# tudocomp/tudocomp

Measured on AMD Instinct MI355X. Metric: input MB/s end-to-end lcpcomp+huffman, higher is better.
Workload: dtype u32; 1 GPU; lcpcomp(coder=huff,threshold=2,flatten=1,comp=arrays) on 2000000000 B english text (SURVEY 8d generator, seed 42): pinned host text -> H2D -> kernels + host Huffman table -> D2H -> stream in pinned host memory, all timed; bytes_per_gpu=2000000000, parallelism=single GPU

## Files before the change

### tudocomp_amd/csrc/api_ctx.hip

```cpp
#include "api.hpp"
#include "huffman_host.hpp"

#include <strings.h>
#include <ctype.h>

using namespace tdc;

namespace tdc {

int lcpcomp_enc_coder(int coder) {
    const int base = coder & 0xFF, k = coder >> 8;
    if (base == TDC_GPU_CODER_SLE) {
        if (k < 0 || k > 7) throw ArgError{TDC_GPU_ERR_ARG, "sle: kmer must be in 1..7"};
        return 3 | ((k ? k : 3) << 8);
    }
    if (k == 0 && base == TDC_GPU_CODER_HUFF) return 0;
    if (k == 0 && base == TDC_GPU_CODER_ARITH) return 1;
    if (k == 0 && base == TDC_GPU_CODER_ASCII) return 2;
    throw ArgError{TDC_GPU_ERR_UNSUPPORTED, "lcpcomp: coder must be huff, arithmetic, ascii or sle"};
}

void reserve_arena(Ctx& c, size_t bytes) {
    if (c.arena.size < bytes) {
        size_t fr = 0, tot = 0;
// ... 23 lines not shown
        case TDC_GPU_ERR_UNSUPPORTED: return "No implementation found for this coder/strategy";
        case TDC_GPU_ERR_INTERNAL: return "internal error";
        default: return "unknown status";
    }
}

const char* tdc_gpu_last_error(const tdc_gpu_ctx* ctx) { return ctx ? ctx->last_error.c_str() : ""; }

void tdc_gpu_free(void* p) { free(p); }

namespace {
struct OptionDef { const char* name; void (*set)(Ctx&, long); };
inline int clampi(long v, long lo, long hi) { return (int)(v < lo ? lo : (v > hi ? hi : v)); }
const OptionDef OPTIONS[] = {
    { "fastread",         [](Ctx& c, long v) { c.fast_read = v ? 1 : 0; } },
    { "sa_local",         [](Ctx& c, long v) { c.sa_local_sort = (int)v; } },
    { "radix_waves",      [](Ctx& c, long v) { c.radix_waves = v == 8 ? 8 : 4; } },
    { "window_lcut",      [](Ctx& c, long v) { c.window_lcut = clampi(v, 0, 63); } },
    { "window_halo",      [](Ctx& c, long v) { c.window_halo = clampi(v, 0, 2048); } },
    { "dec_seg",          [](Ctx& c, long v) { c.dec_seg = v < 4096 ? 4096 : (v > (1l << 30) ? (size_t)1 << 30 : (size_t)v); } },
    { "dec_lean",         [](Ctx& c, long v) { c.dec_lean = v != 0; } },
    { "dec_parse",        [](Ctx& c, long v) { c.dec_parse = clampi(v, 0, 2); } },
    { "dec_done",         [](Ctx& c, long v) { c.dec_done = v != 0; } },
    { "dec_log",          [](Ctx& c, long v) { c.dec_log = v != 0; } },
    { "bwt_log",          [](Ctx& c, long v) { c.bwt_log = v != 0; } },
    { "pipe_log",         [](Ctx& c, long v) { c.pipe_log = v != 0; } },
    { "window_force_fail",[](Ctx& c, long v) { c.window_force_fail = v ? 1 : 0; } },
    { "window_large",     [](Ctx& c, long v) { c.window_large_lists = v ? 1 : 0; } },
    { "window_src",       [](Ctx& c, long v) { c.window_src = v ? 1 : 0; } },
    { "plcp_samples",     [](Ctx& c, long v) { c.plcp_samples = v != 0; } },
    { "small_pipeline",   [](Ctx& c, long v) { c.small_pipeline = v != 0; } },
    { "small_big",        [](Ctx& c, long v) { c.small_big = (int)v; } },
    { "small_prof",       [](Ctx& c, long v) { c.small_prof = v != 0; } },
    { "phi_lazy",         [](Ctx& c, long v) { c.phi_lazy = v != 0; } },
    { "fs_pair",          [](Ctx& c, long v) { c.fs_pair = v != 0; } },
    { "enc_early",        [](Ctx& c, long v) { c.enc_early = (int)v; } },
    { "owner_rem",        [](Ctx& c, long v) { c.owner_rem = (int)std::min<long>(std::max<long>(v, 0), 8); } },
    { "enc_rec",          [](Ctx& c, long v) { c.enc_rec = v != 0; } },
    { "level_purge",      [](Ctx& c, long v) { c.level_purge = v != 0; } },
    { "level_log",        [](Ctx& c, long v) { c.level_log = v != 0; } },
    { "eager",            [](Ctx& c, long v) { c.eager_levels = v != 0; } },
    { "eager_dump",       [](Ctx& c, long v) { c.eager_dump = v != 0; } },
    { "flen_bytes",       [](Ctx& c, long v) { c.flen_bytes = v != 0; } },
    { "flatten_steps",    [](Ctx& c, long v) { c.flatten_steps = v <= 0 ? (1 << 30) : clampi(v, 1, 1 << 30); } },
    { "flatten_growth",   [](Ctx& c, long v) { c.flatten_growth = clampi(v, 2, 1 << 20); } },
    { "sa_refine",        [](Ctx& c, long v) { c.sa_refine = v != 0; } },
    { "sa_pairs",         [](Ctx& c, long v) { c.sa_pairs = v != 0; } },
    { "sa_stars",         [](Ctx& c, long v) { c.sa_stars = v != 0; } },
    { "sa_fused_init",    [](Ctx& c, long v) { c.sa_fused_init = v != 0; } },
    { "sa_init_syms",     [](Ctx& c, long v) { c.sa_init_syms = clampi(v, 0, 64); } },
    { "radix_lds",        [](Ctx& c, long v) { c.radix_lds = (v >= 0 && v <= 2) ? (int)v : 2; } },
    { "xcd_remap",        [](Ctx& c, long v) { c.xcd_remap = (v >= 0 && v <= 2) ? (int)v : 0; } },
    { "bucket_scatter",   [](Ctx& c, long v) { c.bucket_scatter = v ? 1 : 0; } },
    { "ssort",            [](Ctx& c, long v) { c.ssort = v ? 1 : 0; } },
    { "ssort_levels",     [](Ctx& c, long v) { c.ssort_levels = (v >= 1 && v <= 3) ? (int)v : 0; } },
    { "msd_partition",    [](Ctx& c, long v) { c.msd_partition = v ? 1 : 0; } },
    { "wsort",            [](Ctx& c, long v) { c.wsort = v ? 1 : 0; } },
    { "wsort_min",        [](Ctx& c, long v) { c.wsort_min = v < 4096 ? 4096 : (size_t)v; } },
    { "wsort_syms",       [](Ctx& c, long v) { c.wsort_syms = (v >= 4 && v <= 64) ? (int)v : 0; } },
    { "wsort_kw",         [](Ctx& c, long v) { c.wsort_kw = (v == 1 || v == 2) ? (int)v : 0; } },
    { "wsort_rounds",     [](Ctx& c, long v) { c.wsort_rounds = clampi(v, 0, 100); } },
    { "wsort_smallrun",   [](Ctx& c, long v) { c.wsort_small = v ? 1 : 0; } },
    { "wsort_overlap",    [](Ctx& c, long v) { c.wsort_overlap = v ? 1 : 0; } },
    { "wsort_predig",     [](Ctx& c, long v) { c.wsort_predig = v ? 1 : 0; } },
    { "wsort_prehist",    [](Ctx& c, long v) { c.wsort_prehist = v ? 1 : 0; } },
    { "sa_seg_bigcap",    [](Ctx& c, long v) { c.sa_seg_bigcap = clampi(v, 0, 65536); } },
    { "sa_seg_rounds",    [](Ctx& c, long v) { c.sa_seg_rounds = clampi(v, 0, 2); } },
    { "wsort_run_streams",[](Ctx& c, long v) { c.wsort_run_streams = v != 0; } },
    { "wsort_predig_skip",[](Ctx& c, long v) { c.wsort_predig_skip = clampi(v, 0, 24); } },
    { "wsort_fuse",       [](Ctx& c, long v) { c.wsort_fuse = v ? 1 : 0; } },
    { "wsort_order",      [](Ctx& c, long v) { c.wsort_order = v ? 1 : 0; } },
    { "wsort_two",        [](Ctx& c, long v) { c.wsort_two = (v >= 0 && v <= 2) ? (int)v : 0; } },
    { "wsort_leaf",       [](Ctx& c, long v) { c.wsort_leaf = v == 1024 ? 1024 : 2048; } },
    { "wsort_pack",       [](Ctx& c, long v) { c.wsort_pack = (v == 1024 || v == 4096) ? (int)v : 2048; } },
    { "wsort_cmax",       [](Ctx& c, long v) { c.wsort_cmax = clampi(v, 8, 64); } },
    { "wsort_log",        [](Ctx& c, long v) { c.wsort_log = v != 0; } },
    { "upload_chunks",    [](Ctx& c, long v) { c.upload_chunks = clampi(v, 4, 24); } },
    { "upload_tail_n",    [](Ctx& c, long v) { c.upload_tail_n = clampi(v, 0, 12); } },
    { "upload_tail_pct",  [](Ctx& c, long v) { c.upload_tail_pct = clampi(v, 30, 100); } },
    { "arena_log",        [](Ctx& c, long v) { c.arena_log = v != 0; } },
};
constexpr size_t NOPTIONS = sizeof(OPTIONS) / sizeof(OPTIONS[0]);
const OptionDef FOLD_OPTIONS[] = {
    { "fused_cand",       [](Ctx& c, long v) { c.fused_cand = v != 0; } },
    { "sel_tile_counts",  [](Ctx& c, long v) { c.sel_tile_counts = v != 0; } },
    { "flatten_chunks",   [](Ctx& c, long v) { c.flatten_chunks = clampi(v, 0, (long)FLATTEN_MAX_CHUNKS); } },
    { "repair_recount",   [](Ctx& c, long v) { c.repair_recount = v != 0; } },
    { "repair_table_bits",[](Ctx& c, long v) { c.repair_table_bits = v == 0 ? 0 : clampi(v, 8, 30); } },
    { "repair_log",       [](Ctx& c, long v) { c.repair_log = v != 0; } },
};
constexpr size_t NFOLD = sizeof(FOLD_OPTIONS) / sizeof(FOLD_OPTIONS[0]);
const OptionDef* find_option(const char* name) {
    if (!name) return nullptr;
    if (!strncasecmp(name, "TDC_GPU_", 8)) name += 8;
    for (size_t i = 0; i < NOPTIONS; ++i) if (!strcasecmp(name, OPTIONS[i].name)) return &OPTIONS[i];
    for (size_t i = 0; i < NFOLD; ++i) if (!strcasecmp(name, FOLD_OPTIONS[i].name)) return &FOLD_OPTIONS[i];
    return nullptr;
}
void apply_env_options(tdc_gpu_ctx* ctx) {
    const char* on = getenv("TDC_GPU_DEBUG_KNOBS");
    if (!on || atoi(on) == 0) return;
    for (size_t i = 0; i < NOPTIONS + NFOLD; ++i) {
        const OptionDef& o = i < NOPTIONS ? OPTIONS[i] : FOLD_OPTIONS[i - NOPTIONS];
        char var[64] = "TDC_GPU_";
        size_t k = 8;
        for (const char* q = o.name; *q && k + 1 < sizeof(var); ++q) var[k++] = (char)toupper((unsigned char)*q);
        var[k] = 0;
        if (const char* m = getenv(var)) o.set(ctx->c, atol(m));
    }
}
}

int tdc_gpu_ctx_set_option(tdc_gpu_ctx* ctx, const char* name, long value) {
    if (!ctx) return TDC_GPU_ERR_ARG;
    const OptionDef* o = find_option(name);
    if (!o) return TDC_GPU_ERR_ARG;
    o->set(ctx->c, value);
    return TDC_GPU_OK;
}
int tdc_gpu_option_count(void) { return (int)NOPTIONS; }
const char* tdc_gpu_option_name(int i) { return (i >= 0 && (size_t)i < NOPTIONS) ? OPTIONS[i].name : nullptr; }

int tdc_gpu_ctx_create(int device, tdc_gpu_ctx** out) {
    if (!out) return TDC_GPU_ERR_ARG;
    *out = nullptr;
    int count = 0;
    if (hipGetDeviceCount(&count) != hipSuccess || count <= 0) { (void)hipGetLastError(); return TDC_GPU_ERR_HIP; }
    if (device < 0 || device >= count) return TDC_GPU_ERR_ARG;
    tdc_gpu_ctx* ctx = new (std::nothrow) tdc_gpu_ctx();
    if (!ctx) return TDC_GPU_ERR_OOM;
    ctx->c.huff_ok = huffman_selfcheck();
    ctx->c.device = device;
    ctx->c.wpre = &ctx->pre;
    DeviceGuard dg(device);
    try {
        HIP_TRY(dg.enter());
        HIP_TRY(hipStreamCreateWithFlags(&ctx->c.stream, hipStreamNonBlocking));
        for (auto& e : ctx->c.ev) HIP_TRY(hipEventCreate(&e));
        HIP_TRY(hipStreamCreateWithFlags(&ctx->c.copy_stream, hipStreamNonBlocking));
        {
            int lo = 0, hi = 0;
            if (hipDeviceGetStreamPriorityRange(&lo, &hi) != hipSuccess) { lo = 0; (void)hipGetLastError(); }
            if (hipStreamCreateWithPriority(&ctx->c.aux_stream, hipStreamNonBlocking, lo) != hipSuccess) { ctx->c.aux_stream = nullptr; (void)hipGetLastError(); }
        }
        HIP_TRY(hipEventCreateWithFlags(&ctx->c.ev_join, hipEventDisableTiming));
        HIP_TRY(hipEventCreateWithFlags(&ctx->c.ev_dig2, hipEventDisableTiming));
        for (auto& e : ctx->c.ev_chunk) HIP_TRY(hipEventCreateWithFlags(&e, hipEventDisableTiming));
        ctx->c.pinned_size = 4096;
        HIP_TRY(hipHostMalloc(&ctx->c.pinned, ctx->c.pinned_size, hipHostMallocDefault));
        HIP_TRY(hipHostMalloc((void**)&ctx->c.pinned_hdr, Ctx::PINNED_HDR, hipHostMallocDefault));
        if (ctx->c.fast_read) {
            void* zc = nullptr;
            if (hipHostMalloc(&zc, (size_t)Ctx::ZC_WORDS * Ctx::ZC_BLOCKS * 4, hipHostMallocMapped | hipHostMallocCoherent) == hipSuccess) {
                void* dv = nullptr;
                if (hipHostGetDevicePointer(&dv, zc, 0) == hipSuccess) { ctx->c.zc_host = (u32*)zc; ctx->c.zc_dev = (u32*)dv; memset(zc, 0, (size_t)Ctx::ZC_WORDS * Ctx::ZC_BLOCKS * 4); }
                else { (void)hipHostFree(zc); (void)hipGetLastError(); }
            } else (void)hipGetLastError();
        }
        HIP_TRY(hipMalloc((void**)&ctx->c.d_err, 256));
        HIP_TRY(hipMemset(ctx->c.d_err, 0, 256));
        apply_env_options(ctx);
    } catch (const HipError&) {
        (void)hipGetLastError();
        tdc_gpu_ctx_destroy(ctx);
        return TDC_GPU_ERR_HIP;
    }
// ... 142 lines not shown
```

### tudocomp_amd/csrc/common.hpp

```cpp
#pragma once

#include <hip/hip_runtime.h>
#include <stdint.h>
#include <stddef.h>
#include <stdio.h>
#include <string.h>

namespace tdc {

typedef uint8_t  u8;
typedef uint32_t u32;
typedef uint16_t u16;
typedef uint64_t u64;

constexpr u32 NONE32 = 0xFFFFFFFFu;
constexpr int WAVE = 64;

enum {
    TDC_OK = 0,
    TDC_ERR_HIP = -1,
    TDC_ERR_ARG = -2,
    TDC_ERR_NO_SENTINEL = -3,
    TDC_ERR_TOO_LARGE = -4,
    TDC_ERR_OOM = -5,
// ... 44 lines not shown
    }
    template <typename T> T* get_top(size_t count) { return (T*)alloc_top(count * sizeof(T)); }
    void release_top() { top_hi = 0; }
    size_t mark() const { return top; }
    void release(size_t m) { top = m; }
};

enum KernelClass {
    K_RS_SCATTER_U64 = 0, K_RS_SCATTER_U32, K_RS_COUNT, K_SCAN,
    K_SA_RANK_SCATTER, K_SA_BUILD_KEYS, K_PHI, K_PLCP, K_CAND,
    K_LEVEL_INIT, K_MIS_ROUND, K_RESOLVE, K_PUSH, K_APPLY, K_POOL, K_SMALL_LEVEL, K_WINDOW_LEVELS,
    K_FLATTEN_ROUND, K_ENC_GAPS, K_ENC_HIST, K_ENC_TILE_BITS, K_ENC_PACK, K_EXTRACT, K_SS_LEAF, K_SA_LOCAL_SORT, K_WINDOW_SCATTER,
    K_WS_LEAF_SORT, K_WS_LEAF_COUNT, K_WS_RUN, K_FS_IMAGE,
    K_CLASS_COUNT
};

struct KernelProfile {
    double ms = 0;
    u64 launches = 0;
    u64 bytes = 0;
};

#ifdef __HIPCC__
static __global__ void publish_words_kernel(const uint32_t* __restrict__ src, uint32_t nwords, uint32_t* host_dst, uint32_t* host_flag,
                                            uint32_t seq) {
    for (uint32_t i = threadIdx.x; i < nwords; i += blockDim.x)
        __hip_atomic_store(&host_dst[i], src[i], __ATOMIC_RELAXED, __HIP_MEMORY_SCOPE_SYSTEM);
    __syncthreads();
    if (threadIdx.x == 0) {
        __threadfence_system();
        __hip_atomic_store(host_flag, seq, __ATOMIC_RELEASE, __HIP_MEMORY_SCOPE_SYSTEM);
    }
}
#endif

struct Ctx {
    int device = 0;
    hipStream_t stream = nullptr;
    Arena arena;
    hipEvent_t ev[16] = {};
    void* pinned = nullptr;
    size_t pinned_size = 0;
    void* pinned_tab = nullptr;
    size_t pinned_tab_size = 0;
    u8* pinned_hdr = nullptr;
    static constexpr size_t PINNED_HDR = 65536;
    void* pinned_table(size_t bytes) {
        if (pinned_tab_size < bytes) {
            if (pinned_tab) { (void)hipHostFree(pinned_tab); pinned_tab = nullptr; pinned_tab_size = 0; }
            HIP_TRY(hipHostMalloc(&pinned_tab, bytes, hipHostMallocDefault));
            pinned_tab_size = bytes;
        }
        return pinned_tab;
    }
    static constexpr u32 ZC_SEG_OFF = 1040, ZC_WORDS = 1040 + 16384;
    static constexpr u32 ZC_BLOCKS = 3;
    u32* zc_host = nullptr;
    u32* zc_dev = nullptr;
    u32 zc_seq = 0;
    int fast_read = 1;
    u32* d_err = nullptr;
    int sa_local_sort = 1;
    int radix_waves = 4;
    int plcp_samples = 1;
    bool huff_ok = true;
    int flen_bytes = 1;
    int eager_levels = 1;
    int level_purge = 1;
    int enc_rec = 1;
    int owner_rem = 8;
    int enc_early = 1;
    int fused_cand = 1;
    int sel_tile_counts = 1;
    int fs_pair = 1;
    int small_big = 1;
    int small_pipeline = 1;
    int sa_pairs = 1;
    int sa_stars = 1;
    int sa_refine = 1;
    int sa_fused_init = 1;
    int radix_lds = 1;
    int xcd_remap = 1;
    int window_src = 1;
    int window_lcut = 56;
    int window_halo = 320;
    size_t dec_seg = 0;
    bool phi_lazy = true;
    int dec_lean = 1;
    int dec_parse = 1;
    int window_force_fail = 0;
    int window_large_lists = 0;
    int ssort = 1;
    int ssort_levels = 0;
    int wsort = 1;
    size_t wsort_min = (size_t)1 << 20;
    int wsort_syms = 0;
    int wsort_kw = 0;
    int wsort_rounds = 24;
    int wsort_cmax = 24;
    int wsort_overlap = 1;
    int wsort_prehist = 1;
    bool wsort_count_nonheads = true;
    int sa_seg_bigcap = 65536;
    int sa_seg_rounds = 2;
    int wsort_run_streams = 1;
    int wsort_predig_skip = 4;
    int wsort_predig = 1;
    int wsort_two = 0;
    int wsort_leaf = 2048;
    int wsort_pack = 1024;
    int wsort_order = 1;
    int wsort_fuse = 1;
    int wsort_small = 0;
    int msd_partition = 1;
    int bucket_scatter = 1;
    int upload_tail_n = 3, upload_tail_pct = 60;
    int upload_chunks = 16;
    int flatten_steps = 1;
    int flatten_growth = 8;
    int flatten_chunks = 0;
    int sa_init_syms = 0;
    int dec_done = 1;
    int repair_recount = 0;
    int repair_table_bits = 0;
    int repair_log = 0;
    int dec_log = 0, bwt_log = 0, pipe_log = 0, level_log = 0, wsort_log = 0, eager_dump = 0, small_prof = 0, arena_log = 0;

    u32 hist_cache[256] = {};
    const u8* hist_ptr = nullptr;
    size_t hist_n = 0;
    hipStream_t copy_stream = nullptr;
    hipStream_t aux_stream = nullptr;
    hipEvent_t ev_join = nullptr;
    static constexpr size_t CHUNK_EVENTS = 32;
    hipEvent_t ev_chunk[CHUNK_EVENTS] = {};
    hipEvent_t ev_dig2 = nullptr;
    struct WPre* wpre = nullptr;
    u8* d2h_host = nullptr;
    size_t d2h_cap = 0;
    size_t d2h_done = 0;

    bool profiling = false;
    KernelProfile kprof[K_CLASS_COUNT];
    struct Pending { hipEvent_t a, b; int cls; u64 bytes; };
    Pending* pend = nullptr;
    int npend = 0, pend_cap = 0;
    hipEvent_t* ev_pool = nullptr;
    int ev_pool_size = 0, ev_pool_used = 0;

    int prof_begin(int cls, u64 bytes) {
        if (!profiling || npend >= pend_cap || ev_pool_used + 2 > ev_pool_size) return -1;
        Pending& p = pend[npend];
        p.a = ev_pool[ev_pool_used++]; p.b = ev_pool[ev_pool_used++]; p.cls = cls; p.bytes = bytes;
        HIP_TRY(hipEventRecord(p.a, stream));
        return npend++;
    }
    void prof_end(int idx) { if (idx >= 0) HIP_TRY(hipEventRecord(pend[idx].b, stream)); }
    void wait_for(hipStream_t waiter, hipStream_t signaller) {
        HIP_TRY(hipEventRecord(ev_join, signaller));
        HIP_TRY(hipStreamWaitEvent(waiter, ev_join, 0));
    }
    struct ProfScope {
        Ctx& c; int idx;
        ProfScope(Ctx& ctx, int cls, u64 bytes) : c(ctx), idx(ctx.prof_begin(cls, bytes)) {}
        ~ProfScope() { if (idx >= 0) (void)hipEventRecord(c.pend[idx].b, c.stream); }
    };
// ... 279 lines not shown
```

### tudocomp_amd/csrc/factorize_tiles.hip

```cpp
#include "stages.hpp"
#include "prim.hpp"
#include "factorize_tiles.hpp"

#include <stdlib.h>

namespace tdc {

namespace {

#ifndef TDC_WIN_TW
#define TDC_WIN_TW 16384
#endif
#ifndef TDC_WIN_WPE
#define TDC_WIN_WPE 7
#endif
#ifndef TDC_WIN_LB
#define TDC_WIN_LB 4
#endif
#ifndef TDC_WIN_TE
#define TDC_WIN_TE 512
#endif
#ifndef TDC_WIN_TT
#define TDC_WIN_TT 256
#endif
constexpr int TW = TDC_WIN_TW;
constexpr int TH_MAX = 2048;
constexpr int TT = TDC_WIN_TT;
constexpr int TCH = 64;
constexpr int TE_SMALL = TDC_WIN_TE;
constexpr int TE_LARGE = 8192;
#ifndef TDC_WIN_TT_LARGE
#define TDC_WIN_TT_LARGE 1024
#endif
constexpr int TT_LARGE = TDC_WIN_TT_LARGE;

__device__ __forceinline__ int PA(int q) {
    const int t = q >> 6, w = (q >> 2) & 15;
    return (t << 6) + (((w + 2 * (t >> 2)) & 15) << 2) + (q & 3);
}
__device__ __forceinline__ int PW(int t, int k) { return (t << 6) + (((2 * k + 2 * (t >> 2)) & 15) << 2); }
constexpr int BIG = 1 << 29;

enum : u32 { B_VAL = 0x3Fu, B_START = 0x40u, B_TRUNC = 0x80u };
__device__ __forceinline__ u32 b_ub(u32 b) { return (b & B_START) ? 0u : (b & B_VAL); }

enum : u32 { S_UND = 0, S_SEL = 1, S_REJ = 2, S_UNC = 3 };
__device__ __forceinline__ int e_pos(u32 e) { return (int)(e & 0xFFFFu); }
__device__ __forceinline__ u32 e_state(u32 e) { return (e >> 16) & 3u; }
__device__ __forceinline__ u32 e_trunc(u32 e) { return (e >> 18) & 1u; }
__device__ __forceinline__ void e_set_state(u32* ent, int i, u32 e, u32 st) { lds_store(&ent[i], (e & ~(3u << 16)) | (st << 16)); }

struct WinScalars { u32 fail; int min_margin; unsigned long long factors; u32 max_entries, pad; unsigned long long prof[16]; };

#ifdef TDC_WIN_PROF
#define WPROF_DECL unsigned long long wp_t = __builtin_readcyclecounter(); unsigned long long wp_acc[12] = {0,0,0,0,0,0,0,0,0,0,0,0};
#define WPROF(i) do { const unsigned long long wp_n = __builtin_readcyclecounter(); wp_acc[i] += wp_n - wp_t; wp_t = wp_n; } while (0)
#define WPROF_CNT(i, v) do { wp_acc[i] += (v); } while (0)
#define WPROF_FLUSH do { if (tid == 0) for (int wi = 0; wi < 12; ++wi) atomicAdd(&sc->prof[wi], wp_acc[wi]); } while (0)
#define WTRIP(i) do { if (tid < 64) { const u64 wt_a = __ballot(true); if (lane == __builtin_ctzll(wt_a)) atomicAdd(&sc->prof[i], 1ull); } } while (0)
#else
#define WPROF_DECL
#define WPROF(i) do {} while (0)
#define WPROF_CNT(i, v) do {} while (0)
#define WPROF_FLUSH do {} while (0)
#define WTRIP(i) do {} while (0)
#endif

__device__ __forceinline__ void lds_barrier() { asm volatile("s_waitcnt lgkmcnt(0)\n\ts_barrier" ::: "memory"); }

__device__ __forceinline__ u32 hit4(u32 w, u32 pat) {
    const u32 x = (w & 0x7F7F7F7Fu) ^ pat;
    return ~(x + 0x7F7F7F7Fu) & 0x80808080u;
}
template <int KT, int TE, int WPE, int WSRC>
__global__ __launch_bounds__(KT) __attribute__((amdgpu_waves_per_eu(WPE, WPE))) void window_eager_kernel(const u32* __restrict__ cur_g, const u32* __restrict__ prio_g,
                                                            const u8* __restrict__ res_g, const u32* __restrict__ phi, size_t n,
                                                            u32 lcut, u32 threshold, u32 ntiles, u32 halo,
                                                            u32* __restrict__ flen, u8* __restrict__ flen8, u32* __restrict__ fsrc, WinScalars* __restrict__ sc) {
    constexpr int NWV = KT / 64;
    constexpr int CPT = TW / (64 * KT) > 0 ? TW / (64 * KT) : 1;
    static_assert(TW % 64 == 0 && TW / 64 <= KT * CPT, "every chunk of the window needs an owner");
    static_assert(TW <= 65536, "16-bit window positions");
    __shared__ __attribute__((aligned(16))) u8 S[TW];
    __shared__ u32 ent[TE];
    __shared__ u32 pri[TE];
    __shared__ unsigned short selp[NWV][64];
    __shared__ u32 wtot[NWV];
    __shared__ int s_und[3];
    __shared__ int s_tl, s_tr;
    __shared__ u64 s_lvlmask;
    const int tid = threadIdx.x;
    const int lane = tid & 63, wv = tid >> 6;
    WPROF_DECL

    const size_t TH = halo, TI = (size_t)TW - 2 * (size_t)halo;
    for (u32 tile = blockIdx.x; tile < ntiles; tile += gridDim.x) {
        const size_t a = (size_t)tile * TI;
        const size_t b = (a + TI < n) ? a + TI : n;
        const size_t w0 = (a >= (size_t)TH) ? a - TH : 0;
        const size_t w1 = (b + TH < n) ? b + TH : n;
        const int wl = (int)(w1 - w0);
        const int ia = (int)(a - w0), ib = (int)(b - w0);
        const int mid = wl / 2;
        __syncthreads();
        WPROF(0);
        if (tid == 0) { s_und[0] = 0; s_und[1] = 0; s_und[2] = 0; s_tl = -BIG; s_tr = BIG; s_lvlmask = 0; }
        __syncthreads();
        u64 mymask = 0;
        constexpr int LIT = TW / (KT * 4);
        constexpr int LB = LIT < TDC_WIN_LB ? LIT : TDC_WIN_LB;
        static_assert(TW % (KT * 4) == 0 && LIT % LB == 0, "window load");
        if (wl == TW) {
#pragma unroll 1
            for (int it0 = 0; it0 < LIT; it0 += LB) {
                uint4 cv[LB];
                u32 rv4[LB];
                u64 bmask = 0;
#pragma unroll
                for (int u = 0; u < LB; ++u) {
                    const size_t gp = w0 + (size_t)((it0 + u) * KT * 4 + tid * 4);
                    cv[u] = *(const uint4*)(cur_g + gp);
                    rv4[u] = *(const u32*)(res_g + gp);
                }
#pragma unroll
                for (int u = 0; u < LB; ++u) {
                    const int i = (it0 + u) * KT * 4 + tid * 4;
                    const u32 c4[4] = { cv[u].x, cv[u].y, cv[u].z, cv[u].w };
                    u32 sw = 0;
#pragma unroll
                    for (int k = 0; k < 4; ++k) {
                        u32 c = c4[k] > 63u ? 63u : c4[k];
                        if (c < threshold) c = 0;
                        const u32 rv = (rv4[u] >> (8 * k)) & 0xFFu;
                        const u32 bb = c ? (c | (rv != c ? B_TRUNC : 0u)) : 0u;
                        sw |= bb << (8 * k);
                        bmask |= 1ull << c;
                    }
                    *(u32*)&S[PA(i)] = sw;
                }
                mymask |= bmask;
            }
        } else {
            for (int i = tid * 4; i < TW; i += KT * 4) {
                u32 sw = 0;
                const size_t gp = w0 + i;
                if (gp + 4 <= w1) {
                    const uint4 cv = *(const uint4*)(cur_g + gp);
                    const u32 rv4 = *(const u32*)(res_g + gp);
                    const u32 c4[4] = { cv.x, cv.y, cv.z, cv.w };
#pragma unroll
                    for (int k = 0; k < 4; ++k) {
                        u32 c = c4[k] > 63u ? 63u : c4[k];
                        if (c < threshold) c = 0;
                        const u32 rv = (rv4 >> (8 * k)) & 0xFFu;
                        const u32 bb = c ? (c | (rv != c ? B_TRUNC : 0u)) : 0u;
                        sw |= bb << (8 * k);
                        mymask |= 1ull << c;
                    }
                } else {
#pragma unroll
                    for (int k = 0; k < 4; ++k) {
                        if (gp + k < w1) {
                            u32 c = cur_g[gp + k];
                            c = c > 63u ? 63u : c;
                            if (c < threshold) c = 0;
                            const u32 rv = res_g[gp + k];
                            const u32 bb = c ? (c | (rv != c ? B_TRUNC : 0u)) : 0u;
                            sw |= bb << (8 * k);
                            mymask |= 1ull << c;
                            }
                    }
                }
                *(u32*)&S[PA(i)] = sw;
            }
        }
#pragma unroll
        for (int d = 32; d >= 1; d >>= 1) mymask |= __shfl_xor(mymask, d, 64);
        if (lane == 0) atomicOr((unsigned long long*)&s_lvlmask, (unsigned long long)mymask);
        int fl = (w0 > 0) ? (int)lcut - 1 : -BIG;
        int fr = (w1 < n) ? wl - ((int)lcut - 1) : BIG;
        u32 nsel_interior = 0;
        bool failed = false;
        __syncthreads();
        WPROF(1);

        for (u32 L = lcut; L >= threshold && !failed; --L) {
            const int iL = (int)L;
            int dfl = fl, dfr = fr;
            if (fl > -BIG / 2) {
                const int q = fl - 1 - lane;
                const u64 mq = __ballot(lane < iL - 1 && q >= 0 && b_ub(S[PA(q >= 0 ? q : 0)]) >= L);
                if (mq) dfl = fl - 1 - __builtin_ctzll(mq) + iL;
            }
            if (fr < BIG / 2) {
                const int q = fr + lane;
                const u64 mq = __ballot(lane < iL - 1 && q < wl && b_ub(S[PA(q < wl ? q : 0)]) >= L);
                if (mq) dfr = fr + __builtin_ctzll(mq) - (iL - 1);
            }
            const u64 lvl_seen = lds_load(&s_lvlmask);
            if (((lvl_seen >> L) & 1ull) == 0) { fl = dfl; fr = dfr; continue; }
            const int lo = fl > 0 ? fl : 0, hi = fr < wl ? fr : wl;
            u32 alo[CPT], ahi[CPT];
            u32 cnt = 0;
#pragma unroll
            for (int cc = 0; cc < CPT; ++cc) {
                const int chunk = tid * CPT + cc;
                const int base = chunk * TCH;
                u32 ml = 0, mh = 0;
                if (base < TW && base < hi && base + TCH > lo) {
                    const u32 pat = L * 0x01010101u;
                    u64 ws[TCH / 8];
#pragma unroll
                    for (int k = 0; k < TCH / 8; ++k) ws[k] = *(const u64*)&S[PW(chunk, k)];
#pragma unroll
                    for (int k = 0; k < TCH / 8; ++k) {
                        const u32 f = __builtin_amdgcn_udot4(hit4((u32)(ws[k] >> 32), pat), 0x80402010u,
                                                             __builtin_amdgcn_udot4(hit4((u32)ws[k], pat), 0x08040201u, 0u, false), false);
                        const int kk = k & 3;
                        const u32 g = (kk == 0) ? (f >> 7) : (f << (8 * kk - 7));
                        if (k < 4) ml |= g; else mh |= g;
                    }
                    const int rlo = lo - base, rhi = hi - base;
                    if (rlo > 0) { if (rlo >= 32) { ml = 0; mh &= ~((1u << (rlo - 32)) - 1u); } else ml &= ~((1u << rlo) - 1u); }
                    if (rhi < TCH) { if (rhi <= 32) { mh = 0; ml &= (rhi == 32) ? ~0u : ((1u << rhi) - 1u); } else mh &= (1u << (rhi - 32)) - 1u; }
                }
                alo[cc] = ml; ahi[cc] = mh;
                cnt += (u32)__popc(ml) + (u32)__popc(mh);
            }
            WPROF(2);
            const u32 inc = wave_inclusive_sum(cnt);
            if (lane == 63) wtot[wv] = inc;
            lds_barrier();
            u32 off = inc - cnt, total = 0;
#pragma unroll
            for (int k = 0; k < NWV; ++k) { const u32 t = wtot[k]; if (k < wv) off += t; total += t; }
            if (total > (u32)TE) { failed = true; break; }
            const int m = (int)total;
#ifdef TDC_WIN_PROF
            if (tid == 0) atomicMax(&sc->max_entries, total);
#endif
            if (tid == 0) { s_und[0] = m; s_und[1] = 0; s_und[2] = 0; }
#pragma unroll
            for (int cc = 0; cc < CPT; ++cc) {
                u64 amask = ((u64)ahi[cc] << 32) | alo[cc];
                const int base = (tid * CPT + cc) * TCH;
                int p0 = -1, p1 = -1;
                u32 t0 = 0, t1 = 0, r0 = 0, r1 = 0;
                if (amask) { p0 = base + __builtin_ctzll(amask); amask &= amask - 1; t0 = S[PA(p0)] >> 7; }
                if (amask) { p1 = base + __builtin_ctzll(amask); amask &= amask - 1; t1 = S[PA(p1)] >> 7; }
                if (p0 >= 0 && !t0) r0 = prio_g[w0 + p0];
                if (p1 >= 0 && !t1) r1 = prio_g[w0 + p1];
                if (p0 >= 0) { ent[off] = (u32)p0 | (t0 << 18); pri[off] = r0; ++off; }
                if (p1 >= 0) { ent[off] = (u32)p1 | (t1 << 18); pri[off] = r1; ++off; }
                while (amask) {
                    WTRIP(11);
                    const int pos = base + __builtin_ctzll(amask);
                    amask &= amask - 1;
                    const u32 t = S[PA(pos)] >> 7;
                    ent[off] = (u32)pos | (t << 18);
                    pri[off] = t ? 0u : prio_g[w0 + pos];
                    ++off;
                }
            }
            lds_barrier();
            WPROF(3);
            WPROF_CNT(8, 1); WPROF_CNT(9, m);
            if (m == 0) { fl = dfl; fr = dfr; continue; }

            int r = 0;
            for (int guard = 0; guard <= m; ++guard) {
                const int und = lds_load(&s_und[r]);
                if (und == 0) break;
                const int rn = (r + 1) % 3, rc = (r + 2) % 3;
                if (tid == 0) s_und[rc] = 0;
                for (int i = lane * NWV + wv; i < m; i += KT) {
                    WTRIP(12);
                    const u32 e = lds_load(&ent[i]);
                    u32 fL = (i > 0) ? lds_load(&ent[i - 1]) : 0u;
                    u32 fR = (i + 1 < m) ? lds_load(&ent[i + 1]) : 0u;
                    if (e_state(e) != S_UND) continue;
                    const int p = e_pos(e);
                    const u32 et = e_trunc(e);
                    bool hit = false, blocked = false, unc = false;
                    const u32 mypri = pri[i];
                    for (int j = i - 1; j >= 0; --j) {
                        WTRIP(13);
                        const u32 f = (j == i - 1) ? fL : lds_load(&ent[j]);
                        if (p - e_pos(f) >= iL) break;
                        const u32 st = e_state(f);
                        if (st == S_SEL) { hit = true; break; }
                        if (st == S_UND || st == S_UNC) {
                            const bool before = e_trunc(f) ? false : (et ? true : pri[j] < mypri);
                            if (before) { if (st == S_UND) blocked = true; else unc = true; }
                        }
                    }
                    for (int j = i + 1; j < m && !hit; ++j) {
                        WTRIP(14);
                        const u32 f = (j == i + 1) ? fR : lds_load(&ent[j]);
                        if (e_pos(f) - p >= iL) break;
                        const u32 st = e_state(f);
                        if (st == S_SEL) { hit = true; break; }
                        if (st == S_UND || st == S_UNC) {
                            const bool before = e_trunc(f) ? false : (et ? true : pri[j] < mypri);
                            if (before) { if (st == S_UND) blocked = true; else unc = true; }
                        }
                    }
                    if (hit) e_set_state(ent, i, e, S_REJ);
                    else if (!blocked) {
                        const bool exposed = (p < dfl) || (p >= dfr);
                        e_set_state(ent, i, e, (unc || exposed) ? S_UNC : S_SEL);
                    } else {
                        const u64 act = __ballot(true);
                        if (lane == __builtin_ctzll(act)) atomicAdd(&s_und[rn], (int)__popcll(act));
                    }
                }
                lds_barrier();
                r = rn;
                WPROF_CNT(10, 1);
            }
            WPROF(4);
            if (lds_load(&s_und[r]) != 0) { failed = true; break; }

            int G = 1;
            while (G < iL) G <<= 1;
            const int EPB = 64 / G;
            const int gi = lane / G, gj = lane % G;
            u64 newlv = 0;
            for (int pass = 0; pass < 2; ++pass) {
                for (int i0 = 0; i0 < m; i0 += KT) {
                    const int i = i0 + lane * NWV + wv;
                    const bool have = i < m;
                    const u32 e = have ? lds_load(&ent[i]) : 0u;
                    const u32 s = have ? e_state(e) : (u32)S_REJ;
                    const int p = e_pos(e);
                    if (pass == 0 && s == S_UNC) {
                        if (p < mid) atomicMax(&s_tl, p + iL); else atomicMin(&s_tr, p - (iL - 1));
                    }
                    const u64 selm = __ballot(s == S_SEL);
                    if (!selm) continue;
                    const int nsel = (int)__popcll(selm);
                    if (s == S_SEL) lds_store(&selp[wv][__popcll(selm & ((1ull << lane) - 1ull))], (unsigned short)p);
                    __builtin_amdgcn_wave_barrier();
                    for (int b0 = 0; b0 < nsel; b0 += EPB) {
                        WTRIP(15);
                        const int k = b0 + gi;
                        if (k < nsel && gj < iL) {
                            const int ps = (int)lds_load(&selp[wv][k]);
                            if (pass == 0) {
                                const int d = gj + 1, q = ps - d;
                                if (d < iL && q >= 0) {
                                    const u32 bb = S[PA(q)];
                                    if (!(bb & B_START) && (bb & B_VAL) > (u32)d) {
                                        const bool alive = (u32)d >= threshold;
                                        S[PA(q)] = alive ? (u8)(B_TRUNC | (u32)d) : (u8)0;
                                        if (alive) newlv |= 1ull << d;
                                    }
                                }
                            } else {
                                const int q = ps + gj;
                                if (q < wl) S[PA(q)] = (gj == 0) ? (u8)(B_START | L) : (u8)0;
                            }
                        }
                    }
                    __builtin_amdgcn_wave_barrier();
                }
                if (pass == 0) {
                    newlv &= ~lvl_seen;
#pragma unroll
                    for (int d = 32; d >= 1; d >>= 1) newlv |= __shfl_xor(newlv, d, 64);
                    if (lane == 0 && newlv) atomicOr((unsigned long long*)&s_lvlmask, (unsigned long long)newlv);
                    lds_barrier();
                }
            }
            lds_barrier();
            WPROF(5);
            int nfl = dfl, nfr = dfr;
            const int tl = lds_load(&s_tl), tr = lds_load(&s_tr);
            if (tl > nfl) nfl = tl;
            if (tr < nfr) nfr = tr;
            fl = nfl; fr = nfr;
            if (tl > -BIG || tr < BIG) {
                lds_barrier();
                if (tid == 0) { s_tl = -BIG; s_tr = BIG; }
            }
            WPROF(6);
        }
        if (tid == 0 && !failed) {
            int mg = BIG;
            if (fl > -BIG / 2) mg = ia - fl;
            if (fr < BIG / 2 && fr - ib < mg) mg = fr - ib;
            atomicMin(&sc->min_margin, mg);
        }
        if (failed || fl > ia || fr < ib) { if (tid == 0) atomicOr(&sc->fail, failed ? 2u : 1u); }
        else {
#pragma unroll
            for (int cc = 0; cc < CPT; ++cc) {
                const int chunk = tid * CPT + cc;
                const int base = chunk * TCH;
                if (base < TW && base < ib && base + TCH > ia) {
#pragma unroll
                    for (int k = 0; k < TCH; k += 8) {
                        const u64 rw = *(const u64*)&S[PW(chunk, k >> 3)];
                        u64 w = rw & 0x4040404040404040ull;
                        while (w) {
                            const int bb = __builtin_ctzll(w) >> 3;
                            w &= w - 1;
                            const int pos = base + k + bb;
                            if (pos < ia || pos >= ib) continue;
                            const size_t gp = w0 + pos;
                            if (flen8) flen8[gp] = (u8)((rw >> (8 * bb)) & 0x3Fu);
                            else flen[gp] = (u32)(rw >> (8 * bb)) & 0x3Fu;
                            if constexpr (WSRC == 1) fsrc[gp] = phi[gp];
                            else if constexpr (WSRC == 2) { const u32 r = prio_g[gp]; if (r < (u32)n) fsrc[gp] = r ? phi[r - 1] : phi[n - 1]; }
                            ++nsel_interior;
                        }
                    }
                }
            }
        }
        nsel_interior = wave_reduce_sum(nsel_interior);
        if (lane == 0 && nsel_interior) atomicAdd(&sc->factors, (unsigned long long)nsel_interior);
        WPROF(7);
    }
    WPROF_FLUSH;
}

__global__ void window_cleanup_kernel(u32* __restrict__ flen, u8* __restrict__ flen8, size_t n, u32 lcut) {
    const size_t p = (size_t)blockIdx.x * blockDim.x + threadIdx.x;
    if (p >= n) return;
    if (flen8) { if (flen8[p] <= lcut) flen8[p] = 0; }
    else if (flen[p] <= lcut) flen[p] = 0;
}

}

u32 window_levels_max_lcut() { return 63; }
u32 window_levels_window() { return (u32)TW; }
u32 window_levels_small_list() { return (u32)TE_SMALL; }
size_t window_levels_min_text() { return (size_t)4 * TW; }

int factorize_window_levels(Ctx& c, size_t n, const u32* cur, const u32* prio, const u8* res8, const u32* phi, u32 lcut, u32 threshold,
                            FactorSpace fs, u64* nfactors, bool start_large, const u32* src_sa) {
    *nfactors = 0;
    if (lcut < threshold) return 0;
    hipStream_t s = c.stream;
    const size_t mark = c.arena.mark();
    u32 halo = (u32)c.window_halo & ~3u;
    if (halo < 2 * lcut + 64) halo = (2 * lcut + 64 + 3) & ~3u;
    if (halo > (u32)TH_MAX) halo = TH_MAX;
    bool large = c.window_large_lists != 0 || start_large;
    const u32 max_grid = 1u << 20;
    WinScalars* d_sc = (WinScalars*)c.arena.alloc(sizeof(WinScalars));
    WinScalars h;
    int result = 0;
    for (int attempt = 0; attempt < 4; ++attempt) {
        const size_t ti = (size_t)TW - 2 * (size_t)halo;
        const u32 ntiles = cdiv(n, ti);
        const u32 grid = ntiles < max_grid ? ntiles : max_grid;
        HIP_TRY(hipMemsetAsync(d_sc, 0, sizeof(WinScalars), s));
        HIP_TRY(hipMemsetD32Async((hipDeviceptr_t)&d_sc->min_margin, BIG, 1, s));
        {
            Ctx::ProfScope prof(c, K_WINDOW_LEVELS, (u64)((double)n * TW / ti * 5) + (u64)n * 2);
            if (!large) {
                if (phi) window_eager_kernel<TT, TE_SMALL, TDC_WIN_WPE, 1><<<grid, TT, 0, s>>>(cur, prio, res8, phi, n, lcut, threshold, ntiles, halo, fs.flen, fs.flen8, fs.fsrc, d_sc);
                else if (src_sa) window_eager_kernel<TT, TE_SMALL, TDC_WIN_WPE, 2><<<grid, TT, 0, s>>>(cur, prio, res8, src_sa, n, lcut, threshold, ntiles, halo, fs.flen, fs.flen8, fs.fsrc, d_sc);
                else window_eager_kernel<TT, TE_SMALL, TDC_WIN_WPE, 0><<<grid, TT, 0, s>>>(cur, prio, res8, phi, n, lcut, threshold, ntiles, halo, fs.flen, fs.flen8, fs.fsrc, d_sc);
            } else {
                if (phi) window_eager_kernel<TT_LARGE, TE_LARGE, TT_LARGE / 256, 1><<<grid, TT_LARGE, 0, s>>>(cur, prio, res8, phi, n, lcut, threshold, ntiles, halo, fs.flen, fs.flen8, fs.fsrc, d_sc);
                else if (src_sa) window_eager_kernel<TT_LARGE, TE_LARGE, TT_LARGE / 256, 2><<<grid, TT_LARGE, 0, s>>>(cur, prio, res8, src_sa, n, lcut, threshold, ntiles, halo, fs.flen, fs.flen8, fs.fsrc, d_sc);
                else window_eager_kernel<TT_LARGE, TE_LARGE, TT_LARGE / 256, 0><<<grid, TT_LARGE, 0, s>>>(cur, prio, res8, phi, n, lcut, threshold, ntiles, halo, fs.flen, fs.flen8, fs.fsrc, d_sc);
            }
            LAUNCH_CHECK();
        }
        h = c.read(d_sc);
#ifdef TDC_WIN_PROF
        {
            static const char* nm[16] = { "wait_prev", "load", "dense", "scan+write", "select", "apply", "borders", "tail", "levels", "entries", "rounds", "w0 collect3+", "w0 round body", "w0 walk left", "w0 walk right", "w0 apply batch" };
            for (int i = 0; i < 16; ++i) fprintf(stderr, "winprof %-10s %llu\n", nm[i], h.prof[i]);
            fprintf(stderr, "winprof windows %u grid %u attempt %d halo %u min_margin %d fail %u max_entries %u\n", ntiles, grid, attempt,
                    halo, h.min_margin, h.fail, h.max_entries);
        }
#endif
        if (c.level_log) fprintf(stderr, "window pass: attempt %d halo %u lists %s -> fail %u, smallest margin %d\n", attempt, halo, large ? "large" : "small", h.fail, h.min_margin);
        if (c.window_force_fail) h.fail |= 1u;
        result = (int)h.fail;
        if (!h.fail) break;
        window_cleanup_kernel<<<cdiv(n, 256), 256, 0, s>>>(fs.flen, fs.flen8, n, lcut);
        LAUNCH_CHECK();
        bool again = false;
        if ((h.fail & 2u) && !large) { large = true; again = true; }
        if ((h.fail & 1u) && halo < (u32)TH_MAX && !c.window_force_fail) { halo = TH_MAX; again = true; }
        if (!again) break;
    }
    c.arena.release(mark);
    if (result == 0) *nfactors = h.factors;
    return result;
}

}
```

Before: 9070 MB/s.

## Resolve small window levels in a single wave and rotate work across waves

In the window eager factorization kernel, levels with at most 64 candidate entries are now resolved by one wave using wave-local fences instead of block-wide barriers per round. The selected positions are then applied by all waves in a strided batch split. Larger levels deal entries in contiguous 64-wide chunks with a per-tile wave rotation. This is meant to cut block barrier overhead and idle waves in the iterative select loop. It adds code paths and register pressure, and the other waves sit at a barrier while the single wave resolves.

```diff
diff --git a/tudocomp_amd/csrc/api_ctx.hip b/tudocomp_amd/csrc/api_ctx.hip
--- a/tudocomp_amd/csrc/api_ctx.hip
+++ b/tudocomp_amd/csrc/api_ctx.hip
@@ -129,6 +129,7 @@
 };
 constexpr size_t NOPTIONS = sizeof(OPTIONS) / sizeof(OPTIONS[0]);
 const OptionDef FOLD_OPTIONS[] = {
+    { "window_deal",      [](Ctx& c, long v) { c.window_deal = v ? 1 : 0; } },
     { "fused_cand",       [](Ctx& c, long v) { c.fused_cand = v != 0; } },
     { "sel_tile_counts",  [](Ctx& c, long v) { c.sel_tile_counts = v != 0; } },
     { "flatten_chunks",   [](Ctx& c, long v) { c.flatten_chunks = clampi(v, 0, (long)FLATTEN_MAX_CHUNKS); } },
diff --git a/tudocomp_amd/csrc/common.hpp b/tudocomp_amd/csrc/common.hpp
--- a/tudocomp_amd/csrc/common.hpp
+++ b/tudocomp_amd/csrc/common.hpp
@@ -150,6 +150,7 @@
     int radix_lds = 1;
     int xcd_remap = 1;
     int window_src = 1;
+    int window_deal = 1;
     int window_lcut = 56;
     int window_halo = 320;
     size_t dec_seg = 0;
diff --git a/tudocomp_amd/csrc/factorize_tiles.hip b/tudocomp_amd/csrc/factorize_tiles.hip
--- a/tudocomp_amd/csrc/factorize_tiles.hip
+++ b/tudocomp_amd/csrc/factorize_tiles.hip
@@ -50,13 +50,13 @@
 __device__ __forceinline__ u32 e_trunc(u32 e) { return (e >> 18) & 1u; }
 __device__ __forceinline__ void e_set_state(u32* ent, int i, u32 e, u32 st) { lds_store(&ent[i], (e & ~(3u << 16)) | (st << 16)); }
 
-struct WinScalars { u32 fail; int min_margin; unsigned long long factors; u32 max_entries, pad; unsigned long long prof[16]; };
+struct WinScalars { u32 fail; int min_margin; unsigned long long factors; u32 max_entries, pad; unsigned long long prof[24]; };
 
 #ifdef TDC_WIN_PROF
-#define WPROF_DECL unsigned long long wp_t = __builtin_readcyclecounter(); unsigned long long wp_acc[12] = {0,0,0,0,0,0,0,0,0,0,0,0};
+#define WPROF_DECL unsigned long long wp_t = __builtin_readcyclecounter(); unsigned long long wp_acc[24] = {};
 #define WPROF(i) do { const unsigned long long wp_n = __builtin_readcyclecounter(); wp_acc[i] += wp_n - wp_t; wp_t = wp_n; } while (0)
 #define WPROF_CNT(i, v) do { wp_acc[i] += (v); } while (0)
-#define WPROF_FLUSH do { if (tid == 0) for (int wi = 0; wi < 12; ++wi) atomicAdd(&sc->prof[wi], wp_acc[wi]); } while (0)
+#define WPROF_FLUSH do { if (tid == 0) for (int wi = 0; wi < 24; ++wi) if (wp_acc[wi]) atomicAdd(&sc->prof[wi], wp_acc[wi]); } while (0)
 #define WTRIP(i) do { if (tid < 64) { const u64 wt_a = __ballot(true); if (lane == __builtin_ctzll(wt_a)) atomicAdd(&sc->prof[i], 1ull); } } while (0)
 #else
 #define WPROF_DECL
@@ -67,12 +67,13 @@
 #endif
 
 __device__ __forceinline__ void lds_barrier() { asm volatile("s_waitcnt lgkmcnt(0)\n\ts_barrier" ::: "memory"); }
+__device__ __forceinline__ void wave_lds_fence() { asm volatile("s_waitcnt lgkmcnt(0)" ::: "memory"); __builtin_amdgcn_wave_barrier(); }
 
 __device__ __forceinline__ u32 hit4(u32 w, u32 pat) {
     const u32 x = (w & 0x7F7F7F7Fu) ^ pat;
     return ~(x + 0x7F7F7F7Fu) & 0x80808080u;
 }
-template <int KT, int TE, int WPE, int WSRC>
+template <int KT, int TE, int WPE, int WSRC, int DEAL>
 __global__ __launch_bounds__(KT) __attribute__((amdgpu_waves_per_eu(WPE, WPE))) void window_eager_kernel(const u32* __restrict__ cur_g, const u32* __restrict__ prio_g,
                                                             const u8* __restrict__ res_g, const u32* __restrict__ phi, size_t n,
                                                             u32 lcut, u32 threshold, u32 ntiles, u32 halo,
@@ -239,7 +240,8 @@
 #ifdef TDC_WIN_PROF
             if (tid == 0) atomicMax(&sc->max_entries, total);
 #endif
-            if (tid == 0) { s_und[0] = m; s_und[1] = 0; s_und[2] = 0; }
+            const bool one_wave = DEAL != 0 && m <= 64;
+            if (tid == 0) { s_und[0] = one_wave ? 0 : m; s_und[1] = 0; s_und[2] = 0; }
 #pragma unroll
             for (int cc = 0; cc < CPT; ++cc) {
                 u64 amask = ((u64)ahi[cc] << 32) | alo[cc];
@@ -265,20 +267,10 @@
             lds_barrier();
             WPROF(3);
             WPROF_CNT(8, 1); WPROF_CNT(9, m);
+            WPROF_CNT(m == 0 ? 16 : m <= 64 ? 17 : m <= 128 ? 18 : m <= 256 ? 19 : 20, 1);
             if (m == 0) { fl = dfl; fr = dfr; continue; }
 
-            int r = 0;
-            for (int guard = 0; guard <= m; ++guard) {
-                const int und = lds_load(&s_und[r]);
-                if (und == 0) break;
-                const int rn = (r + 1) % 3, rc = (r + 2) % 3;
-                if (tid == 0) s_und[rc] = 0;
-                for (int i = lane * NWV + wv; i < m; i += KT) {
-                    WTRIP(12);
-                    const u32 e = lds_load(&ent[i]);
-                    u32 fL = (i > 0) ? lds_load(&ent[i - 1]) : 0u;
-                    u32 fR = (i + 1 < m) ? lds_load(&ent[i + 1]) : 0u;
-                    if (e_state(e) != S_UND) continue;
+            auto decide = [&](const int i, const u32 e, const u32 fL, const u32 fR) -> u32 {
                     const int p = e_pos(e);
                     const u32 et = e_trunc(e);
                     bool hit = false, blocked = false, unc = false;
@@ -305,47 +297,22 @@
                             if (before) { if (st == S_UND) blocked = true; else unc = true; }
                         }
                     }
-                    if (hit) e_set_state(ent, i, e, S_REJ);
-                    else if (!blocked) {
-                        const bool exposed = (p < dfl) || (p >= dfr);
-                        e_set_state(ent, i, e, (unc || exposed) ? S_UNC : S_SEL);
-                    } else {
-                        const u64 act = __ballot(true);
-                        if (lane == __builtin_ctzll(act)) atomicAdd(&s_und[rn], (int)__popcll(act));
-                    }
-                }
-                lds_barrier();
-                r = rn;
-                WPROF_CNT(10, 1);
-            }
-            WPROF(4);
-            if (lds_load(&s_und[r]) != 0) { failed = true; break; }
-
+                    if (hit) return (u32)S_REJ;
+                    if (blocked) return (u32)S_UND;
+                    const bool exposed = (p < dfl) || (p >= dfr);
+                    return (unc || exposed) ? (u32)S_UNC : (u32)S_SEL;
+            };
             int G = 1;
             while (G < iL) G <<= 1;
             const int EPB = 64 / G;
             const int gi = lane / G, gj = lane % G;
             u64 newlv = 0;
-            for (int pass = 0; pass < 2; ++pass) {
-                for (int i0 = 0; i0 < m; i0 += KT) {
-                    const int i = i0 + lane * NWV + wv;
-                    const bool have = i < m;
-                    const u32 e = have ? lds_load(&ent[i]) : 0u;
-                    const u32 s = have ? e_state(e) : (u32)S_REJ;
-                    const int p = e_pos(e);
-                    if (pass == 0 && s == S_UNC) {
-                        if (p < mid) atomicMax(&s_tl, p + iL); else atomicMin(&s_tr, p - (iL - 1));
-                    }
-                    const u64 selm = __ballot(s == S_SEL);
-                    if (!selm) continue;
-                    const int nsel = (int)__popcll(selm);
-                    if (s == S_SEL) lds_store(&selp[wv][__popcll(selm & ((1ull << lane) - 1ull))], (unsigned short)p);
-                    __builtin_amdgcn_wave_barrier();
-                    for (int b0 = 0; b0 < nsel; b0 += EPB) {
+            auto apply_batches = [&](const int pass, const int nsel, const unsigned short* list, const int first, const int step) {
+                    for (int b0 = first * EPB; b0 < nsel; b0 += step * EPB) {
                         WTRIP(15);
                         const int k = b0 + gi;
                         if (k < nsel && gj < iL) {
-                            const int ps = (int)lds_load(&selp[wv][k]);
+                            const int ps = (int)lds_load(&list[k]);
                             if (pass == 0) {
                                 const int d = gj + 1, q = ps - d;
                                 if (d < iL && q >= 0) {
@@ -362,18 +329,113 @@
                             }
                         }
                     }
-                    __builtin_amdgcn_wave_barrier();
-                }
-                if (pass == 0) {
+            };
+            auto publish_levels = [&]() {
                     newlv &= ~lvl_seen;
 #pragma unroll
                     for (int d = 32; d >= 1; d >>= 1) newlv |= __shfl_xor(newlv, d, 64);
                     if (lane == 0 && newlv) atomicOr((unsigned long long*)&s_lvlmask, (unsigned long long)newlv);
+            };
+            const int rot = DEAL ? (int)((L + tile) % (u32)NWV) : 0;
+            const int sw = (wv - rot + NWV) % NWV;
+
+            if (one_wave) {
+                if (wv == rot) {
+                    const bool have = lane < m;
+                    const u32 e = have ? lds_load(&ent[lane]) : 0u;
+                    u32 s = S_REJ;
+                    bool und = have;
+                    for (int guard = 0; guard <= m; ++guard) {
+                        if (!__ballot(und)) break;
+                        if (und) {
+                            WTRIP(12);
+                            const u32 fL = (lane > 0) ? lds_load(&ent[lane - 1]) : 0u;
+                            const u32 fR = (lane + 1 < m) ? lds_load(&ent[lane + 1]) : 0u;
+                            const u32 ns = decide(lane, e, fL, fR);
+                            if (ns != S_UND) { e_set_state(ent, lane, e, ns); s = ns; und = false; }
+                        }
+                        wave_lds_fence();
+                        WPROF_CNT(10, 1);
+                    }
+                    if (wv == 0) WPROF(4);
+                    if (__ballot(und)) { if (lane == 0) lds_store(&s_und[0], 1); }
+                    else {
+                        const int p = e_pos(e);
+                        if (s == S_UNC) {
+                            if (p < mid) atomicMax(&s_tl, p + iL); else atomicMin(&s_tr, p - (iL - 1));
+                        }
+                        const u64 selm = __ballot(s == S_SEL);
+                        if (selm) {
+                            const int nsel = (int)__popcll(selm);
+                            if (s == S_SEL) lds_store(&selp[0][__popcll(selm & ((1ull << lane) - 1ull))], (unsigned short)p);
+                            if (lane == 0) lds_store(&s_und[1], nsel);
+                        }
+                    }
+                }
+                lds_barrier();
+                const int nsel = lds_load(&s_und[1]);
+                if (nsel > 0 && lds_load(&s_und[0]) == 0) {
+                    apply_batches(0, nsel, selp[0], sw, NWV);
+                    publish_levels();
+                    lds_barrier();
+                    apply_batches(1, nsel, selp[0], sw, NWV);
+                }
+                lds_barrier();
+                WPROF(5);
+                if (lds_load(&s_und[0]) != 0) { failed = true; break; }
+            } else {
+            int r = 0;
+            for (int guard = 0; guard <= m; ++guard) {
+                const int und = lds_load(&s_und[r]);
+                if (und == 0) break;
+                const int rn = (r + 1) % 3, rc = (r + 2) % 3;
+                if (tid == 0) s_und[rc] = 0;
+                for (int i = DEAL ? sw * 64 + lane : lane * NWV + wv; i < m; i += KT) {
+                    WTRIP(12);
+                    const u32 e = lds_load(&ent[i]);
+                    const u32 fL = (i > 0) ? lds_load(&ent[i - 1]) : 0u;
+                    const u32 fR = (i + 1 < m) ? lds_load(&ent[i + 1]) : 0u;
+                    if (e_state(e) != S_UND) continue;
+                    const u32 ns = decide(i, e, fL, fR);
+                    if (ns != S_UND) e_set_state(ent, i, e, ns);
+                    else {
+                        const u64 act = __ballot(true);
+                        if (lane == __builtin_ctzll(act)) atomicAdd(&s_und[rn], (int)__popcll(act));
+                    }
+                }
+                lds_barrier();
+                r = rn;
+                WPROF_CNT(10, 1);
+            }
+            WPROF(4);
+            if (lds_load(&s_und[r]) != 0) { failed = true; break; }
+
+            for (int pass = 0; pass < 2; ++pass) {
+                for (int i0 = 0; i0 < m; i0 += KT) {
+                    const int i = i0 + lane * NWV + wv;
+                    const bool have = i < m;
+                    const u32 e = have ? lds_load(&ent[i]) : 0u;
+                    const u32 s = have ? e_state(e) : (u32)S_REJ;
+                    const int p = e_pos(e);
+                    if (pass == 0 && s == S_UNC) {
+                        if (p < mid) atomicMax(&s_tl, p + iL); else atomicMin(&s_tr, p - (iL - 1));
+                    }
+                    const u64 selm = __ballot(s == S_SEL);
+                    if (!selm) continue;
+                    const int nsel = (int)__popcll(selm);
+                    if (s == S_SEL) lds_store(&selp[wv][__popcll(selm & ((1ull << lane) - 1ull))], (unsigned short)p);
+                    __builtin_amdgcn_wave_barrier();
+                    apply_batches(pass, nsel, selp[wv], 0, 1);
+                    __builtin_amdgcn_wave_barrier();
+                }
+                if (pass == 0) {
+                    publish_levels();
                     lds_barrier();
                 }
             }
             lds_barrier();
             WPROF(5);
+            }
             int nfl = dfl, nfr = dfr;
             const int tl = lds_load(&s_tl), tr = lds_load(&s_tr);
             if (tl > nfl) nfl = tl;
@@ -430,6 +492,20 @@
     if (p >= n) return;
     if (flen8) { if (flen8[p] <= lcut) flen8[p] = 0; }
     else if (flen[p] <= lcut) flen[p] = 0;
+}
+
+template <int DEAL>
+void launch_window(hipStream_t s, u32 grid, bool large, const u32* cur, const u32* prio, const u8* res8, const u32* phi, const u32* src_sa, size_t n,
+                   u32 lcut, u32 threshold, u32 ntiles, u32 halo, const FactorSpace& fs, WinScalars* d_sc) {
+    if (!large) {
+        if (phi) window_eager_kernel<TT, TE_SMALL, TDC_WIN_WPE, 1, DEAL><<<grid, TT, 0, s>>>(cur, prio, res8, phi, n, lcut, threshold, ntiles, halo, fs.flen, fs.flen8, fs.fsrc, d_sc);
+        else if (src_sa) window_eager_kernel<TT, TE_SMALL, TDC_WIN_WPE, 2, DEAL><<<grid, TT, 0, s>>>(cur, prio, res8, src_sa, n, lcut, threshold, ntiles, halo, fs.flen, fs.flen8, fs.fsrc, d_sc);
+        else window_eager_kernel<TT, TE_SMALL, TDC_WIN_WPE, 0, DEAL><<<grid, TT, 0, s>>>(cur, prio, res8, phi, n, lcut, threshold, ntiles, halo, fs.flen, fs.flen8, fs.fsrc, d_sc);
+    } else {
+        if (phi) window_eager_kernel<TT_LARGE, TE_LARGE, TT_LARGE / 256, 1, DEAL><<<grid, TT_LARGE, 0, s>>>(cur, prio, res8, phi, n, lcut, threshold, ntiles, halo, fs.flen, fs.flen8, fs.fsrc, d_sc);
+        else if (src_sa) window_eager_kernel<TT_LARGE, TE_LARGE, TT_LARGE / 256, 2, DEAL><<<grid, TT_LARGE, 0, s>>>(cur, prio, res8, src_sa, n, lcut, threshold, ntiles, halo, fs.flen, fs.flen8, fs.fsrc, d_sc);
+        else window_eager_kernel<TT_LARGE, TE_LARGE, TT_LARGE / 256, 0, DEAL><<<grid, TT_LARGE, 0, s>>>(cur, prio, res8, phi, n, lcut, threshold, ntiles, halo, fs.flen, fs.flen8, fs.fsrc, d_sc);
+    }
 }
 
 }
@@ -461,22 +537,16 @@
         HIP_TRY(hipMemsetD32Async((hipDeviceptr_t)&d_sc->min_margin, BIG, 1, s));
         {
             Ctx::ProfScope prof(c, K_WINDOW_LEVELS, (u64)((double)n * TW / ti * 5) + (u64)n * 2);
-            if (!large) {
-                if (phi) window_eager_kernel<TT, TE_SMALL, TDC_WIN_WPE, 1><<<grid, TT, 0, s>>>(cur, prio, res8, phi, n, lcut, threshold, ntiles, halo, fs.flen, fs.flen8, fs.fsrc, d_sc);
-                else if (src_sa) window_eager_kernel<TT, TE_SMALL, TDC_WIN_WPE, 2><<<grid, TT, 0, s>>>(cur, prio, res8, src_sa, n, lcut, threshold, ntiles, halo, fs.flen, fs.flen8, fs.fsrc, d_sc);
-                else window_eager_kernel<TT, TE_SMALL, TDC_WIN_WPE, 0><<<grid, TT, 0, s>>>(cur, prio, res8, phi, n, lcut, threshold, ntiles, halo, fs.flen, fs.flen8, fs.fsrc, d_sc);
-            } else {
-                if (phi) window_eager_kernel<TT_LARGE, TE_LARGE, TT_LARGE / 256, 1><<<grid, TT_LARGE, 0, s>>>(cur, prio, res8, phi, n, lcut, threshold, ntiles, halo, fs.flen, fs.flen8, fs.fsrc, d_sc);
-                else if (src_sa) window_eager_kernel<TT_LARGE, TE_LARGE, TT_LARGE / 256, 2><<<grid, TT_LARGE, 0, s>>>(cur, prio, res8, src_sa, n, lcut, threshold, ntiles, halo, fs.flen, fs.flen8, fs.fsrc, d_sc);
-                else window_eager_kernel<TT_LARGE, TE_LARGE, TT_LARGE / 256, 0><<<grid, TT_LARGE, 0, s>>>(cur, prio, res8, phi, n, lcut, threshold, ntiles, halo, fs.flen, fs.flen8, fs.fsrc, d_sc);
-            }
+            if (c.window_deal) launch_window<1>(s, grid, large, cur, prio, res8, phi, src_sa, n, lcut, threshold, ntiles, halo, fs, d_sc);
+            else launch_window<0>(s, grid, large, cur, prio, res8, phi, src_sa, n, lcut, threshold, ntiles, halo, fs, d_sc);
             LAUNCH_CHECK();
         }
         h = c.read(d_sc);
 #ifdef TDC_WIN_PROF
         {
-            static const char* nm[16] = { "wait_prev", "load", "dense", "scan+write", "select", "apply", "borders", "tail", "levels", "entries", "rounds", "w0 collect3+", "w0 round body", "w0 walk left", "w0 walk right", "w0 apply batch" };
-            for (int i = 0; i < 16; ++i) fprintf(stderr, "winprof %-10s %llu\n", nm[i], h.prof[i]);
+            static const char* nm[21] = { "wait_prev", "load", "dense", "scan+write", "select", "apply+wait", "borders", "tail", "levels", "entries", "rounds", "w0 collect3+", "w0 round body", "w0 walk left", "w0 walk right", "w0 apply batch",
+                                          "levels m=0", "levels m<=64", "levels m<=128", "levels m<=256", "levels m>256" };
+            for (int i = 0; i < 21; ++i) fprintf(stderr, "winprof %-14s %llu\n", nm[i], h.prof[i]);
             fprintf(stderr, "winprof windows %u grid %u attempt %d halo %u min_margin %d fail %u max_entries %u\n", ntiles, grid, attempt,
                     halo, h.min_margin, h.fail, h.max_entries);
         }
```

Result: no change. 9126 MB/s, median of 6 (+0.6%).
